# dmosopt/dmosopt

Hardware: NVIDIA H100
Metric: candidate-evals/sec (GP+sort+HV) pop=65536 dim=30 obj=3 (higher is better)
Workload: dtype f64 results; GP variance contraction in split-fp16 wgmma with fp32 accumulation (precision=auto: calibrated against the float64 path, 0 of 65535 rows of the last step recomputed in float64); ranks on u32 ids

## Files before the change

dmosopt_b200/csrc/common.cuh:

```cuda
#pragma once

#include <cuda_runtime.h>
#include <math.h>
#include <stdint.h>
#include <stdio.h>

#include <string>
#include <vector>

#include "../../include/dmosopt_b200.h"

struct dmo_ctx {
  int device = 0;
  cudaStream_t stream = nullptr;
  cudaMemPool_t pool = nullptr;
  cudaEvent_t ev0 = nullptr, ev1 = nullptr;
  int sm_count = 132;
  int64_t launches = 0;
  int64_t waits = 0;
  std::string err;
  void* flush_buf = nullptr;
  size_t flush_bytes = 0;
  int* dev_flag = nullptr;
  uint64_t h2d_bytes = 0, d2h_bytes = 0;
// ... 210 lines not shown
};
__device__ __forceinline__ double u01_53(uint32_t hi, uint32_t lo) {
  return (double)((((uint64_t)(hi >> 5)) << 26) | (uint64_t)(lo >> 6)) * (1.0 / 9007199254740992.0);
}

__device__ __forceinline__ double warp_sum(double v) {
#pragma unroll
  for (int o = 16; o > 0; o >>= 1) v += __shfl_xor_sync(0xffffffffu, v, o);
  return v;
}

template <int NW>
__device__ __forceinline__ double block_sum(double v, double* red) {
  v = warp_sum(v);
  __syncthreads();
  if ((threadIdx.x & 31) == 0) red[threadIdx.x >> 5] = v;
  __syncthreads();
  double s = 0.0;
#pragma unroll 8
  for (int w = 0; w < NW; ++w) s += red[w];
  __syncthreads();
  return s;
}

#endif

int prim_sort_pairs_u64(dmo_ctx* ctx, const uint64_t* kin, uint64_t* kout, const uint32_t* vin,
                        uint32_t* vout, int64_t n, int begin_bit, int end_bit);
int prim_sort_pairs_u32(dmo_ctx* ctx, const uint32_t* kin, uint32_t* kout, const uint32_t* vin,
                        uint32_t* vout, int64_t n, int begin_bit, int end_bit);
int prim_inclusive_sum_u32(dmo_ctx* ctx, const uint32_t* in, uint32_t* out, int64_t n);
int prim_exclusive_sum_i32(dmo_ctx* ctx, const int32_t* in, int32_t* out, int64_t n);
int prim_inclusive_min_f64(dmo_ctx* ctx, const double* in, double* out, int64_t n);
int prim_iota_u32(dmo_ctx* ctx, uint32_t* out, int64_t n);
int prim_gather_u32(dmo_ctx* ctx, const uint32_t* src, const uint32_t* idx, int64_t n, uint32_t* out);
int prim_round_f32(dmo_ctx* ctx, double* a, int64_t n);
int prim_col_keys(dmo_ctx* ctx, const double* dF, int64_t n, int M, int j, uint64_t* keys, uint32_t* idx);
int prim_sort_by_column(dmo_ctx* ctx, const double* dF, int64_t n, int M, int j, DevBuf<uint32_t>& sidx);

int rank_nd_device(dmo_ctx* ctx, const double* dY, int64_t n, int M, int32_t* d_rank);
int rank_nd_device_keep(dmo_ctx* ctx, const double* dY, int64_t n, int M, int64_t keep, int32_t* d_rank);
int nondominated_flags_device(dmo_ctx* ctx, const double* dY, int64_t n, int M, int32_t* d_flag01);
int nondominated_keep_flags(dmo_ctx* ctx, const double* dF, int64_t n, int M, DevBuf<int32_t>& flag);
int dense_ids(dmo_ctx* ctx, const double* dY, int64_t n, int M, DevBuf<uint32_t>& R, DevBuf<uint32_t>& maxid);
int lex_order(dmo_ctx* ctx, const uint32_t* R, int64_t n, int M, int sshift, DevBuf<uint32_t>& permA, DevBuf<uint32_t>& permB,
              const uint32_t** perm);
int crowding_device(dmo_ctx* ctx, const double* dY, int64_t n, int M, double* dD);
int euclidean_device(dmo_ctx* ctx, const double* dY, int64_t n, int M, double* dD);
int lexsort_device(dmo_ctx* ctx, const int32_t* d_rank, const double* const* d_desc_keys, int nkeys,
                   int64_t n, uint32_t* d_perm, bool rank_below_n);
int hypervolume_device(dmo_ctx* ctx, const double* dF, int64_t n, int M, const double* h_ref, double* h_out);
int hypervolume_device_ranked(dmo_ctx* ctx, const double* dF, int64_t n, int M, const double* h_ref, const int32_t* d_rank,
                              double* h_out);
int tournament_device(dmo_ctx* ctx, const int32_t* d_rank, const double* d_crowd, int64_t pop, int64_t poolsize, uint64_t seed,
                      uint64_t stream_id, int64_t* d_pool, double* d_u);
int nsga2_generate_device(dmo_ctx* ctx, const double* d_pop_x, int d, const int64_t* d_pool, int64_t poolsize, int64_t popsize,
                          double crossover_prob, double mutation_prob, double mutation_rate, const double* d_dic,
                          const double* d_dim, const double* d_xlb, const double* d_xub, uint64_t seed, uint64_t stream_id,
                          double* d_x_gen, int32_t* d_kind, int64_t* n_children, double* d_draws);
int remove_worst_device(dmo_ctx* ctx, const double* dX, const double* dY, int64_t n, int d, int M, int metric,
                        const double* const* d_extra, int n_extra, int64_t keep, double* dX_out, double* dY_out, int32_t* d_rank_out,
                        int64_t* d_perm_out);
int feas_rank_device(dmo_ctx* ctx, const dmo_feas* m, const double* dX, int64_t n, double* d_rank);
int feas_model_dim(const dmo_feas* m);
```

dmosopt_b200/csrc/gp.cuh:

```cuda
#pragma once
#include <vector>

#include "common.cuh"

struct GpVarOps {
  int64_t Npad = 0;
  int G = 0;
  std::vector<double> h_kscale;
  DevBuf<double> Linv;
  bool tensor_ready = false;
  DevBuf<uint16_t> Lhi, Llo;
  DevBuf<float> Lscale;
  DevBuf<int> Kexp;
  int alloc(dmo_ctx* ctx, int64_t N, int G);
};

struct dmo_gp {
  int64_t N = 0;
  int d = 0, M = 0, kernel = 0;
  bool isotropic = true;
  GpVarOps ops;
  std::vector<int> h_cov, h_lead;
  DevBuf<int> cov;
  DevBuf<double> Xt;
  DevBuf<double> alpha;
  DevBuf<double> inv_ls;
  DevBuf<double> g_inv_ls, g_constant;
  DevBuf<double> constant, noise, ymean, ystd;
  DevBuf<double> xlb, xrg;
  std::vector<double> h_constant, h_noise, h_ystd;
  bool has_linear_mean = false;
  DevBuf<double> lin_w, lin_b;
  DevBuf<float> Xtf;
  DevBuf<float> CAf;
  bool calibrated = false;
  bool auto_mean_tensor = false;
  bool auto_var_tensor = false;
  double cal_mean_err = 0.0;
  bool auto_mean_only = false;
  double cal_mean_err_only = 0.0;
  double cal_var_err = 0.0;
  double refine_theta = 1.0;
  int64_t last_refined = 0;
};

__device__ __forceinline__ double stationary(double s2, int kind) {
  if (kind == DMO_KERNEL_MATERN52) {
    const double K = sqrt(s2) * 2.23606797749978969641;
    return (1.0 + K + K * K / 3.0) * exp(-K);
  }
  return exp(-0.5 * s2);
}

constexpr int64_t GP_MAX_CHUNK = (int64_t)1 << 20;

int gp_predict_fp64(dmo_ctx* ctx, dmo_gp* gp, const double* dXn, int64_t P, double* d_mean, double* d_var);

int gp_linv_from_factor(dmo_ctx* ctx, const double* L, int64_t N, int64_t ldo, double* dst);
int gp_linv_from_factor_batched(dmo_ctx* ctx, const double* L, int64_t ldl, int64_t sL, int64_t N, int nbat, int64_t ldo,
                                int64_t sdst, double* dst);
int gp_fit_batched(dmo_ctx* ctx, int64_t N, int d, int nbat, int kernel, const double* X, const double* inv_ls, const double* constant,
                   const double* diag_add, const double* y, double* A, int64_t ld, int* info, double* work, double* alpha, double* lml);
int gp_potrf_batched(dmo_ctx* ctx, double* A, int64_t ld, int nbat, int* info);
constexpr int GP_F64_TILE = 128;
int gp_var_contract_fp64(dmo_ctx* ctx, const GpVarOps& ops, const double* Ks, int64_t kplane, int64_t Pcpad, int nsplit,
                         double* vnorm, int64_t vn_ld);
int gp_prepare_tensor(dmo_ctx* ctx, GpVarOps& ops);
constexpr int GP_TC_TILE = 128;
int gp_tensor_var_planes(int64_t Npad);
int gp_var_contract_tensor(dmo_ctx* ctx, const GpVarOps& ops, const uint16_t* Kh, const uint16_t* Kl, int64_t k_alloc,
                           int64_t k_rows, int64_t Pcpad, double* vnorm, int64_t vn_ld, int* abort_flag);
struct GpOverlap {
  cudaEvent_t mean_ready = nullptr;
};
int gp_predict_tensor(dmo_ctx* ctx, dmo_gp* gp, const double* dXn, int64_t P, double* d_mean, double* d_var,
                      int* abort_flag = nullptr, const GpOverlap* ov = nullptr);
extern const char* const GP_WATCHDOG_MSG;
struct GpPending {
  GpOverlap ov;
  bool active = false;
  int64_t P = 0;
  const double* dXn = nullptr;
  double *d_mean = nullptr, *d_var = nullptr;
  DevBuf<double> xn;
  DevBuf<int32_t> flag, pos;
};
int gp_predict_device(dmo_ctx* ctx, dmo_gp* gp, const double* dX, int64_t P, double* d_mean, double* d_var, int precision,
                      GpPending* pending = nullptr);
int gp_predict_finish(dmo_ctx* ctx, dmo_gp* gp, GpPending& pending, bool* refined);

struct GpUnitPredict {
  const char* who = "";
  bool tensor = false;
  int64_t tile = 0;
  int64_t Pc_alloc = 0;
  int n_vp = 0;
  DevBuf<double> vnorm, Ks;
  DevBuf<uint16_t> Kh, Kl;
  DevBuf<int> abort_flag;
  int check(dmo_ctx* ctx, const char* who, int precision, int d);
  int alloc(dmo_ctx* ctx, int64_t P, int64_t Npad, int planes, bool want_var);
  int contract(dmo_ctx* ctx, const GpVarOps& ops, int64_t Pcpad);
  int watchdog(dmo_ctx* ctx);
};

template <typename T>
int upload(dmo_ctx* ctx, DevBuf<T>& dst, const std::vector<T>& src) {
  DMO_TRY(dst.alloc(ctx, src.size()));
  DMO_CUDA(cudaMemcpyAsync(dst.p, src.data(), src.size() * sizeof(T), cudaMemcpyHostToDevice, ctx->stream));
  return DMO_OK;
}

int sv_gemm(dmo_ctx* ctx, int64_t m, int64_t n, int64_t K, double alpha, const double* A, int64_t sai, int64_t sak, const double* B,
            int64_t sbk, int64_t sbj, double diag, double* C, int64_t ldc);
int sv_flip(dmo_ctx* ctx, const double* C, int64_t n, double s, double* O, int64_t ldo);
int svgp_latent_moments(dmo_ctx* ctx, dmo_svgp* sv, GpUnitPredict& up, const double* X, int64_t P, double* fm, double* fv);
struct SvLatentView {
  const double *O0, *O1, *A, *XtT, *inv_ls;
  int64_t Npad;
};
int svgp_latent_view(const dmo_svgp* sv, int l, SvLatentView* v);

constexpr int MT_MAX = 8;
constexpr int MT_FIT_DMAX = 90;
// ... 26 lines not shown
```

dmosopt_b200/csrc/gp_tensor.cu:

```cuda
#include <cuda.h>
#include <cuda_fp16.h>
#include <cudaTypedefs.h>
#include <stdlib.h>

#include "gp.cuh"

namespace {

constexpr int TN = 256;
constexpr int TMV = 128;
constexpr int TK = 32;
constexpr int UK = 16;
constexpr int STAGES = 4;
constexpr int A_BYTES = TMV * TK * 2;
constexpr int B_BYTES = TN * TK * 2;
constexpr int STAGE_BYTES = 2 * A_BYTES + 2 * B_BYTES;
constexpr size_t GEMM_SMEM = (size_t)STAGES * STAGE_BYTES + 1024 + 256;
constexpr int NTHREADS = 384;

__device__ __forceinline__ uint32_t smem_u32(const void* p) { return (uint32_t)__cvta_generic_to_shared(p); }

__device__ __forceinline__ void mbar_init(uint64_t* bar, uint32_t count) {
  asm volatile("mbarrier.init.shared::cta.b64 [%0], %1;" ::"r"(smem_u32(bar)), "r"(count) : "memory");
}
// ... 846 lines not shown
#define KM_SWITCH(ISO_)        \
  switch (M) {                 \
    case 1: KM_LAUNCH(ISO_, 1); break; \
    case 2: KM_LAUNCH(ISO_, 2); break; \
    case 3: KM_LAUNCH(ISO_, 3); break; \
    case 4: KM_LAUNCH(ISO_, 4); break; \
    case 5: KM_LAUNCH(ISO_, 5); break; \
    default: KM_LAUNCH(ISO_, 6); break; \
  }
      if (gp->isotropic) {
        KM_SWITCH(true)
      } else {
        KM_SWITCH(false)
      }
#undef KM_SWITCH
#undef KM_LAUNCH
    }
    DMO_LAUNCH(mean_finish_tc_kernel, (unsigned)ceil_div(Pc * M, 256), 256, 0, mpart.p, (int)nsplit, Pc, ld, M, gp->ymean.p,
               gp->ystd.p, p_base, d_mean);
  }
  DMO_CHECK_LAUNCH();
  return DMO_OK;
}

}

int gp_prepare_tensor(dmo_ctx* ctx, GpVarOps& ops) {
  if (ops.tensor_ready) return DMO_OK;
  const int G = ops.G;
  const int64_t Npad = ops.Npad;
  std::vector<int> kexp(G);
  for (int g = 0; g < G; ++g) {
    double c = ops.h_kscale[g];
    kexp[g] = (c > 0.0) ? 13 - ilogb(c) : 13;
  }
  DMO_TRY(ops.Kexp.alloc(ctx, G));
  DMO_CUDA(cudaMemcpyAsync(ops.Kexp.p, kexp.data(), G * sizeof(int), cudaMemcpyHostToDevice, ctx->stream));
  DMO_CUDA(dmo_wait(ctx));
  DMO_TRY(ops.Lhi.alloc(ctx, (size_t)G * Npad * Npad));
  DMO_TRY(ops.Llo.alloc(ctx, (size_t)G * Npad * Npad));
  DMO_TRY(ops.Lscale.alloc(ctx, (size_t)G * Npad));
  DMO_LAUNCH(split_linv_kernel, (unsigned)(G * Npad), 256, 0, ops.Linv.p, Npad, ops.Kexp.p, ops.Lhi.p, ops.Llo.p,
             ops.Lscale.p);
  DMO_CHECK_LAUNCH();
  ops.tensor_ready = true;
  return DMO_OK;
}

static_assert(TMV == GP_TC_TILE, "gp.cuh exports the wgmma candidate tile");

int gp_tensor_var_planes(int64_t Npad) { return (int)((Npad / TN + 1) / 2); }

int gp_var_contract_tensor(dmo_ctx* ctx, const GpVarOps& ops, const uint16_t* Kh, const uint16_t* Kl, int64_t k_alloc,
                           int64_t k_rows, int64_t Pcpad, double* vnorm, int64_t vn_ld, int* abort_flag) {
  const int64_t Npad = ops.Npad;
  DMO_REQUIRE(Npad % TN == 0 && Pcpad % TMV == 0, "gp_var_contract_tensor: internal padding error");
  CUtensorMap map_kh, map_kl, map_lh, map_ll;
  DMO_TRY(make_map(ctx, &map_kh, Kh, (uint64_t)k_alloc, (uint64_t)Npad, TMV, TK, CU_TENSOR_MAP_SWIZZLE_64B));
  DMO_TRY(make_map(ctx, &map_kl, Kl, (uint64_t)k_alloc, (uint64_t)Npad, TMV, TK, CU_TENSOR_MAP_SWIZZLE_64B));
  DMO_TRY(make_map(ctx, &map_lh, ops.Lhi.p, (uint64_t)ops.G * Npad, (uint64_t)Npad, TN, TK, CU_TENSOR_MAP_SWIZZLE_64B));
  DMO_TRY(make_map(ctx, &map_ll, ops.Llo.p, (uint64_t)ops.G * Npad, (uint64_t)Npad, TN, TK, CU_TENSOR_MAP_SWIZZLE_64B));
  DMO_CUDA(cudaFuncSetAttribute(gp_var_wgmma_kernel, cudaFuncAttributeMaxDynamicSharedMemorySize, (int)GEMM_SMEM));
  GemmParams prm;
  prm.M = ops.G;
  prm.n_pb = (int)(Pcpad / TMV);
  prm.n_jt = (int)(Npad / TN);
  prm.n_q = gp_tensor_var_planes(Npad);
  prm.k_rows = k_rows;
  prm.l_rows = Npad;
  prm.inv_scale = ops.Lscale.p;
  prm.vnorm = vnorm;
  prm.vn_ld = vn_ld;
  prm.abort_flag = abort_flag;
  const int n_work = prm.M * prm.n_pb * prm.n_q;
  const int per_cta = (int)ceil_div(n_work, ctx->sm_count);
  const int grid = (int)ceil_div(n_work, per_cta);
  DMO_LAUNCH(gp_var_wgmma_kernel, grid, NTHREADS, GEMM_SMEM, map_kh, map_kl, map_lh, map_ll, prm);
  return DMO_OK;
}

const char* const GP_WATCHDOG_MSG = "gp_predict(tensor): pipeline watchdog tripped (mbarrier wait timed out)";

int gp_predict_tensor(dmo_ctx* ctx, dmo_gp* gp, const double* dXn, int64_t P, double* d_mean, double* d_var, int* abort_flag,
                      const GpOverlap* ov) {
  const int64_t N = gp->N, Npad = gp->ops.Npad;
  const int M = gp->M, G = gp->ops.G, d = gp->d;
  DMO_REQUIRE(M <= 16, "gp_predict(tensor): at most 16 objectives per model (got %d)", M);
  DMO_REQUIRE(d <= 64, "gp_predict(tensor): at most 64 input dimensions (got %d); use DMO_GP_FP64", d);
  DMO_REQUIRE(Npad % TN == 0, "gp_predict(tensor): internal padding error");
  if (!d_var && d <= KM_D && M <= 6)
    return gp_mean_direct(ctx, gp, dXn, P, d_mean);
  DMO_TRY(gp_prepare_tensor(ctx, gp->ops));
  constexpr int64_t TMv = KM_Q;
  int64_t Pc_max = ((int64_t)6 << 30) / ((int64_t)G * Npad * 4);
  if (Pc_max > GP_MAX_CHUNK) Pc_max = GP_MAX_CHUNK;
  Pc_max = (Pc_max / TMv) * TMv;
  if (Pc_max < TMv) Pc_max = TMv;
  const int64_t Pc_alloc = P < Pc_max ? ceil_div(P, TMv) * TMv : Pc_max;
  const int n_q = gp_tensor_var_planes(Npad);
  DevBuf<uint16_t> Kh, Kl;
  DevBuf<double> vnorm;
  DevBuf<int> own_flag;
  DMO_TRY(Kh.alloc(ctx, (size_t)G * Pc_alloc * Npad));
  DMO_TRY(Kl.alloc(ctx, (size_t)G * Pc_alloc * Npad));
  DMO_TRY(vnorm.alloc(ctx, (size_t)n_q * G * Pc_alloc));
  const bool read_back = abort_flag == nullptr;
  if (read_back) {
    DMO_TRY(own_flag.alloc(ctx, 1));
    abort_flag = own_flag.p;
  }
  DMO_CUDA(cudaMemsetAsync(abort_flag, 0, sizeof(int), ctx->stream));
  const int64_t kplane = Pc_alloc * Npad;
  const bool fused = d <= KM_D && M <= 6 && (gp->isotropic || G <= 2) &&
                     !(getenv("DMO_GP_FUSED") && atoi(getenv("DMO_GP_FUSED")) == 0);
  DevBuf<double> mpart;
  if (fused) DMO_TRY(prepare_direct_state(ctx, gp));
  for (int64_t p_base = 0; p_base < P; p_base += Pc_alloc) {
    const int64_t Pc = (P - p_base) < Pc_alloc ? (P - p_base) : Pc_alloc;
    const int64_t Pcpad = ceil_div(Pc, TMv) * TMv;
    if (fused) {
      int64_t n_per_block = Npad;
      const int64_t n_qb = Pcpad / KM_Q;
      const int64_t nsplit = pick_slices(n_qb, Npad, KF_NS, (int64_t)3 * ctx->sm_count, &n_per_block);
      DMO_TRY(mpart.alloc(ctx, (size_t)nsplit * M * Pcpad));
      dim3 gf((unsigned)nsplit, (unsigned)(Pcpad / KS_Q));
      const size_t smem = kstar_mean_smem(M);
      {
        ProfileScope ps_(ctx, "gp_kstar");
// ... 21 lines not shown
      case 4: KF_LAUNCH(ISO_, 4, false); break;                 \
      case 5: KF_LAUNCH(ISO_, 5, false); break;                 \
      default: KF_LAUNCH(ISO_, 6, false); break;                \
    }                                                           \
  }
        if (gp->isotropic) {
          KF_SWITCH(true)
        } else {
          KF_SWITCH(false)
        }
#undef KF_SWITCH
#undef KF_LAUNCH
      }
      DMO_LAUNCH(mean_finish_tc_kernel, (unsigned)ceil_div(Pc * M, 256), 256, 0, mpart.p, (int)nsplit, Pc, Pcpad, M, gp->ymean.p,
                 gp->ystd.p, p_base, d_mean);
    } else {
      {
        ProfileScope ps_(ctx, "gp_kstar");
        const int dmax = d <= 32 ? 32 : 64;
        size_t smem = (size_t)(KT_TP * dmax + G * dmax + G) * sizeof(float);
        dim3 gk((unsigned)(Npad / (2 * KT_TN)), (unsigned)ceil_div(Pcpad, KT_TP));
#define KSTAR_LAUNCH(ISO_, DM_)                                                                                          \
  DMO_LAUNCH((kstar_tensor_kernel<ISO_, DM_>), gk, KT_TN, smem, dXn, P, p_base, Pcpad, gp->Xt.p, N, d, G, gp->kernel, \
             gp->g_inv_ls.p, gp->g_constant.p, gp->ops.Kexp.p, Npad, kplane, Kh.p, Kl.p)
        if (gp->isotropic) {
          if (d <= 32)
            KSTAR_LAUNCH(true, 32);
          else
            KSTAR_LAUNCH(true, 64);
        } else {
          if (d <= 32)
            KSTAR_LAUNCH(false, 32);
          else
            KSTAR_LAUNCH(false, 64);
        }
#undef KSTAR_LAUNCH
      }
      {
        ProfileScope ps_(ctx, "gp_mean");
        DMO_LAUNCH(mean_split_kernel, (unsigned)ceil_div(Pc * M * 32, 256), 256, 0, Kh.p, Kl.p, Pc, N, Npad, kplane, M,
                   gp->cov.p, gp->ops.Kexp.p, gp->alpha.p, gp->ymean.p, gp->ystd.p, p_base, d_mean);
      }
    }
    if (ov && p_base + Pc_alloc >= P) DMO_CUDA(cudaEventRecord(ov->mean_ready, ctx->stream));
    if (d_var) {
      {
        ProfileScope ps_(ctx, "gp_var");
        cudaStream_t main = ctx->stream;
        if (ov) {
          DMO_CUDA(cudaEventRecord(ctx->lane_ev[1], main));
          DMO_CUDA(cudaStreamWaitEvent(ctx->gp_hi, ctx->lane_ev[1], 0));
          ctx->stream = ctx->gp_hi;
        }
        const int rc = gp_var_contract_tensor(ctx, gp->ops, Kh.p, Kl.p, G * Pc_alloc, Pc_alloc, Pcpad, vnorm.p, Pc_alloc, abort_flag);
        if (ov) {
          ctx->stream = main;
          DMO_CUDA(cudaEventRecord(ctx->lane_ev[2], ctx->gp_hi));
          DMO_CUDA(cudaStreamWaitEvent(main, ctx->lane_ev[2], 0));
        }
        DMO_TRY(rc);
      }
      DMO_LAUNCH(var_finish_tc_kernel, (unsigned)ceil_div(Pc * M, 256), 256, 0, vnorm.p, n_q, Pc, Pc_alloc, M, G,
                 gp->cov.p, gp->constant.p, gp->noise.p, gp->ystd.p, p_base, d_var);
    }
  }
  DMO_CHECK_LAUNCH();
  if (!read_back) return DMO_OK;
  int h_abort = 0;
  DMO_CUDA(cudaMemcpyAsync(&h_abort, abort_flag, sizeof(int), cudaMemcpyDeviceToHost, ctx->stream));
  DMO_CUDA(dmo_wait(ctx));
  if (h_abort) return dmo_fail(ctx, DMO_ERR_INTERNAL, "%s", GP_WATCHDOG_MSG);
  return DMO_OK;
}
```

dmosopt_b200/csrc/hv.cu:

```cuda
#include <stdlib.h>

#include "common.cuh"

int hv_many_device(dmo_ctx* ctx, const double* Fnd, const uint32_t* sidx, int64_t n, int M, const double* dref, double* h_out);
int hv3_tree_device(dmo_ctx* ctx, const double* xs, const double* ys, const double* zs, const uint32_t* zo, int64_t n, double rx,
                    double ry, double rz, double* partial, int64_t* n_partial);

namespace {

constexpr int HV_T = 128;

__global__ void inside_flag_kernel(const double* __restrict__ F, int64_t n, int M, const double* __restrict__ ref,
                                   const int32_t* __restrict__ drop, int32_t* __restrict__ flag) {
  int64_t i = (int64_t)blockIdx.x * blockDim.x + threadIdx.x;
  if (i > n) return;
  if (i == n) {
    flag[i] = 0;
    return;
  }
  bool in = drop == nullptr || drop[i] == 0;
  for (int j = 0; j < M; ++j) in = in && (ref[j] > F[i * M + j]);
  flag[i] = in ? 1 : 0;
}

__global__ void rank0_flag_kernel(const int32_t* __restrict__ rank, int64_t n, int32_t* __restrict__ flag) {
  int64_t i = (int64_t)blockIdx.x * blockDim.x + threadIdx.x;
  if (i > n) return;
  flag[i] = (i < n && rank[i] == 0) ? 1 : 0;
}

__global__ void compact_rows_kernel(const double* __restrict__ F, int64_t n, int M, const int32_t* __restrict__ flag,
                                    const int32_t* __restrict__ pos, double* __restrict__ out) {
  int64_t i = (int64_t)blockIdx.x * blockDim.x + threadIdx.x;
  if (i >= n || !flag[i]) return;
  for (int j = 0; j < M; ++j) out[(int64_t)pos[i] * M + j] = F[i * M + j];
}

__global__ void invert_perm_kernel(const uint32_t* __restrict__ sidx, int64_t n, uint32_t* __restrict__ inv) {
  int64_t p = (int64_t)blockIdx.x * blockDim.x + threadIdx.x;
  if (p < n) inv[sidx[p]] = (uint32_t)p;
}

__global__ void min_col_kernel(const double* __restrict__ F, int64_t n, double* out) {
  __shared__ double s[256];
  double m = INFINITY;
  for (int64_t i = threadIdx.x; i < n; i += blockDim.x) m = fmin(m, F[i]);
  s[threadIdx.x] = m;
  __syncthreads();
  for (int o = 128; o > 0; o >>= 1) {
    if (threadIdx.x < o) s[threadIdx.x] = fmin(s[threadIdx.x], s[threadIdx.x + o]);
    __syncthreads();
  }
  if (threadIdx.x == 0) out[0] = s[0];
// ... 322 lines not shown
                 int64_t* count) {
  DevBuf<int32_t> pos;
  DMO_TRY(pos.alloc(ctx, n + 1));
  DMO_TRY(prim_exclusive_sum_i32(ctx, flag.p, pos.p, n + 1));
  int32_t h = 0;
  DMO_CUDA(cudaMemcpyAsync(&h, pos.p + n, sizeof(int32_t), cudaMemcpyDeviceToHost, ctx->stream));
  DMO_CUDA(dmo_wait(ctx));
  *count = h;
  DMO_TRY(out.alloc(ctx, (size_t)(h > 0 ? h : 1) * M));
  if (h > 0) DMO_LAUNCH(compact_rows_kernel, (unsigned)ceil_div(n, 256), 256, 0, dF, n, M, flag.p, pos.p, out.p);
  DMO_CHECK_LAUNCH();
  return DMO_OK;
}

}

int nondominated_keep_flags(dmo_ctx* ctx, const double* dF, int64_t n, int M, DevBuf<int32_t>& flag) {
  DevBuf<uint32_t> sidx;
  DMO_TRY(flag.alloc(ctx, n + 1));
  if (n >= 1024) {
    DevBuf<int32_t> rank;
    DMO_TRY(rank.alloc(ctx, n));
    DMO_TRY(nondominated_flags_device(ctx, dF, n, M, rank.p));
    DMO_LAUNCH(rank0_flag_kernel, (unsigned)ceil_div(n + 1, 256), 256, 0, rank.p, n, flag.p);
    return DMO_OK;
  }
  DMO_TRY(prim_sort_by_column(ctx, dF, n, M, 0, sidx));
  {
    ProfileScope ps(ctx, "nd_filter");
    if (M <= 8)
      DMO_LAUNCH(nondominated_flag_kernel<8>, (unsigned)ceil_div(n, ND_T), ND_T, (size_t)ND_T * M * sizeof(double), dF, sidx.p, n, M,
                 flag.p);
    else
      DMO_LAUNCH(nondominated_flag_kernel<16>, (unsigned)ceil_div(n, ND_T), ND_T, (size_t)ND_T * M * sizeof(double), dF, sidx.p, n, M,
                 flag.p);
  }
  return DMO_OK;
}

namespace {

int nondominated_subset(dmo_ctx* ctx, const double* dF, int64_t n, int M, DevBuf<double>& out, int64_t* count) {
  DevBuf<int32_t> flag;
  DMO_TRY(nondominated_keep_flags(ctx, dF, n, M, flag));
  DMO_TRY(compact_rows(ctx, dF, n, M, flag, out, count));
  return DMO_OK;
}

__global__ void dominated_flag_kernel(const int32_t* __restrict__ keep, int64_t n, int32_t* __restrict__ out) {
  int64_t i = (int64_t)blockIdx.x * blockDim.x + threadIdx.x;
  if (i < n) out[i] = keep[i] ? 0 : 1;
}

int sum_partials(dmo_ctx* ctx, DevBuf<double>& partial, int64_t nb, double* h_out) {
  DevBuf<double> res;
  DMO_TRY(res.alloc(ctx, 1));
  DMO_LAUNCH(final_sum_kernel, 1, 256, 0, partial.p, nb, res.p);
  DMO_CHECK_LAUNCH();
  DMO_CUDA(cudaMemcpyAsync(h_out, res.p, sizeof(double), cudaMemcpyDeviceToHost, ctx->stream));
  DMO_CUDA(dmo_wait(ctx));
  return DMO_OK;
}

}

int hv_inside_nondominated(dmo_ctx* ctx, const double* dF, int64_t n, int M, const double* dref, DevBuf<double>& out,
                           int64_t* count) {
  *count = 0;
  DevBuf<int32_t> flag;
  DevBuf<double> Fin;
  int64_t n1 = 0;
  DMO_TRY(flag.alloc(ctx, n + 1));
  DMO_LAUNCH(inside_flag_kernel, (unsigned)ceil_div(n + 1, 256), 256, 0, dF, n, M, dref, (const int32_t*)nullptr, flag.p);
  DMO_TRY(compact_rows(ctx, dF, n, M, flag, Fin, &n1));
  if (n1 == 0) return DMO_OK;
  return nondominated_subset(ctx, Fin.p, n1, M, out, count);
}

int hypervolume_device_ranked(dmo_ctx* ctx, const double* dF, int64_t n, int M, const double* h_ref, const int32_t* d_rank,
                              double* h_out);

int hypervolume_device(dmo_ctx* ctx, const double* dF, int64_t n, int M, const double* h_ref, double* h_out) {
  return hypervolume_device_ranked(ctx, dF, n, M, h_ref, nullptr, h_out);
}

int hypervolume_device_ranked(dmo_ctx* ctx, const double* dF, int64_t n, int M, const double* h_ref, const int32_t* d_rank,
                              double* h_out) {
  *h_out = 0.0;
  if (n <= 0) return DMO_OK;
  DMO_REQUIRE(M >= 1 && M <= 8, "hypervolume: M=%d not supported (1..8; >= 10 objectives use Monte-Carlo in the reference)", M);
  DevBuf<double> dref;
  DMO_TRY(dref.alloc(ctx, M));
  DMO_CUDA(cudaMemcpyAsync(dref.p, h_ref, M * sizeof(double), cudaMemcpyHostToDevice, ctx->stream));
  DevBuf<int32_t> flag;
  DevBuf<double> Fin;
  int64_t n1 = 0;
  DMO_TRY(flag.alloc(ctx, n + 1));
  DMO_LAUNCH(inside_flag_kernel, (unsigned)ceil_div(n + 1, 256), 256, 0, dF, n, M, dref.p, d_rank, flag.p);
  DMO_TRY(compact_rows(ctx, dF, n, M, flag, Fin, &n1));
  if (n1 == 0) return DMO_OK;
  if (M == 1) {
    DevBuf<double> mn;
    DMO_TRY(mn.alloc(ctx, 1));
    DMO_LAUNCH(min_col_kernel, 1, 256, 0, Fin.p, n1, mn.p);
    DMO_CHECK_LAUNCH();
    double h = 0.0;
// ... 53 lines not shown
    for (int a = 0; a < D; ++a) {
      DMO_TRY(sc[a].alloc(ctx, n2));
      DMO_TRY(so_[a].alloc(ctx, n2));
      DMO_TRY(prim_sort_by_column(ctx, Fnd.p, n2, M, 2 + a, sidx_a));
      DMO_LAUNCH(invert_perm_kernel, g4, 256, 0, sidx_a.p, n2, inv_a.p);
      DMO_TRY(prim_gather_u32(ctx, inv_a.p, sx.p, n2, so_[a].p));
      DMO_LAUNCH(gather_col_kernel, g4, 256, 0, Fnd.p, sx.p, n2, M, 2 + a, sc[a].p);
      A.s[a] = sc[a].p;
      A.o[a] = so_[a].p;
      A.rs[a] = h_ref[2 + a];
    }
    const int64_t tiles = ceil_div(n2, HV_T);
    const int64_t nbv = ceil_div(n2, 256);
    DevBuf<double> part_main, part_a, part_b;
    DMO_TRY(part_main.alloc(ctx, (size_t)n2 * tiles));
    DMO_TRY(part_a.alloc(ctx, nbv));
    DMO_TRY(part_b.alloc(ctx, nbv));
    DMO_REQUIRE(tiles <= 65535, "hypervolume: front too large for M=%d (%lld non-dominated points)", M, (long long)n2);
    dim3 grid((unsigned)n2, (unsigned)tiles);
    double t_main = 0.0, t_a = 0.0, t_b = 0.0;
    {
      ProfileScope ps(ctx, M == 4 ? "hv4" : "hv5");
      if (M == 4) {
        DMO_LAUNCH(hv_slice_kernel<2>, grid, HV_T, 0, A, n2, part_main.p);
        DMO_LAUNCH(hv_volume_terms_kernel<2>, (unsigned)nbv, 256, 0, A, n2, part_a.p, part_b.p);
      } else {
        DMO_LAUNCH(hv_slice_kernel<3>, grid, HV_T, 0, A, n2, part_main.p);
        DMO_LAUNCH(hv_volume_terms_kernel<3>, (unsigned)nbv, 256, 0, A, n2, part_a.p, part_b.p);
      }
    }
    DMO_TRY(sum_partials(ctx, part_main, n2 * tiles, &t_main));
    DMO_TRY(sum_partials(ctx, part_a, nbv, &t_a));
    if (M == 5) DMO_TRY(sum_partials(ctx, part_b, nbv, &t_b));
    *h_out = (M == 4) ? (t_a - t_main) : (t_a - t_b + t_main);
    return DMO_OK;
  }
  DevBuf<uint32_t> sz, zinv, zo;
  DevBuf<double> xs, ys, zs;
  DMO_TRY(prim_sort_by_column(ctx, Fnd.p, n2, M, 2, sz));
  DMO_TRY(zinv.alloc(ctx, n2));
  DMO_TRY(zo.alloc(ctx, n2));
  DMO_TRY(xs.alloc(ctx, n2));
  DMO_TRY(ys.alloc(ctx, n2));
  DMO_TRY(zs.alloc(ctx, n2));
  const unsigned g = (unsigned)ceil_div(n2, 256);
  DMO_LAUNCH(invert_perm_kernel, g, 256, 0, sz.p, n2, zinv.p);
  DMO_TRY(prim_gather_u32(ctx, zinv.p, sx.p, n2, zo.p));
  DMO_LAUNCH(gather_col_kernel, g, 256, 0, Fnd.p, sx.p, n2, M, 0, xs.p);
  DMO_LAUNCH(gather_col_kernel, g, 256, 0, Fnd.p, sx.p, n2, M, 1, ys.p);
  DMO_LAUNCH(gather_col_kernel, g, 256, 0, Fnd.p, sx.p, n2, M, 2, zs.p);
  int64_t nb = ceil_div(n2, HV_T);
  DevBuf<double> partial;
  DMO_TRY(partial.alloc(ctx, nb));
  int64_t tree_min = 4096;
  if (const char* e = getenv("DMO_HV3_TREE")) {
    const long v = atol(e);
    tree_min = v == 0 ? INT64_MAX : (v == 1 ? 0 : v);
  }
  if (n2 >= tree_min) {
    DMO_TRY(hv3_tree_device(ctx, xs.p, ys.p, zs.p, zo.p, n2, h_ref[0], h_ref[1], h_ref[2], partial.p, &nb));
  } else {
    ProfileScope ps(ctx, "hv3");
    DMO_LAUNCH(hv3_kernel, (unsigned)nb, HV_T, 0, xs.p, ys.p, zs.p, zo.p, n2, h_ref[0], h_ref[1], h_ref[2], partial.p);
  }
  DMO_TRY(sum_partials(ctx, partial, nb, h_out));
  return DMO_OK;
}

extern "C" {

int dmo_hypervolume(dmo_ctx* ctx, const double* F, int64_t n, int M, const double* ref, double* out) {
  if (!ctx) return DMO_ERR_ARG;
  DMO_CUDA(cudaSetDevice(ctx->device));
  DMO_REQUIRE(out && ref && n >= 0 && M >= 1 && M <= 16, "hypervolume: bad arguments");
  *out = 0.0;
  if (n == 0) return DMO_OK;
  DMO_REQUIRE(F, "hypervolume: null points");
  double h_ref[16];
  DMO_CUDA(cudaMemcpy(h_ref, ref, M * sizeof(double), cudaMemcpyDefault));
  In<double> f;
  DMO_TRY(f.init(ctx, F, (size_t)n * M));
  DMO_TRY(hypervolume_device(ctx, f.d, n, M, h_ref, out));
  return DMO_OK;
}

int dmo_nondominated_flags(dmo_ctx* ctx, const double* Y, int64_t n, int M, int32_t* flags) {
  if (!ctx) return DMO_ERR_ARG;
  DMO_CUDA(cudaSetDevice(ctx->device));
  DMO_REQUIRE(n >= 0 && M >= 1 && M <= 16, "nondominated_flags: bad shape n=%lld M=%d", (long long)n, M);
  if (n == 0) return DMO_OK;
  DMO_REQUIRE(Y && flags, "nondominated_flags: null pointer");
  In<double> y;
  Out<int32_t> f;
  DMO_TRY(y.init(ctx, Y, (size_t)n * M));
  DMO_TRY(f.init(ctx, flags, (size_t)n));
  DevBuf<int32_t> keep;
  DMO_TRY(nondominated_keep_flags(ctx, y.d, n, M, keep));
  DMO_LAUNCH(dominated_flag_kernel, (unsigned)ceil_div(n, 256), 256, 0, keep.p, n, f.d);
  DMO_CHECK_LAUNCH();
  DMO_TRY(f.finish(ctx));
  DMO_CUDA(dmo_wait(ctx));
  return DMO_OK;
}

int dmo_hypervolume_ranked(dmo_ctx* ctx, const double* F, int64_t n, int M, const double* ref, const int32_t* rank,
                           double* out) {
  if (!ctx) return DMO_ERR_ARG;
  DMO_CUDA(cudaSetDevice(ctx->device));
  DMO_REQUIRE(out && ref && n >= 0 && M >= 1 && M <= 16, "hypervolume_ranked: bad arguments");
  *out = 0.0;
  if (n == 0) return DMO_OK;
  DMO_REQUIRE(F && rank, "hypervolume_ranked: null points / ranks");
  double h_ref[16];
  DMO_CUDA(cudaMemcpy(h_ref, ref, M * sizeof(double), cudaMemcpyDefault));
  In<double> f;
  In<int32_t> r;
  DMO_TRY(f.init(ctx, F, (size_t)n * M));
  DMO_TRY(r.init(ctx, rank, (size_t)n));
  DMO_TRY(hypervolume_device_ranked(ctx, f.d, n, M, h_ref, r.d, out));
// ... 71 lines not shown
```

dmosopt_b200/csrc/step.cu:

```cuda
#include <string.h>

#include <algorithm>

#include "common.cuh"
#include "gp.cuh"

constexpr int kCountWarps = 8;
__global__ void __launch_bounds__(kCountWarps * 32) step_counts_kernel(const int32_t* __restrict__ kind, int64_t P,
                                                                        const int64_t* __restrict__ perm, int64_t pop,
                                                                        unsigned long long* counts) {
  __shared__ double red[kCountWarps];
  double c[4] = {0.0, 0.0, 0.0, 0.0};
  const int64_t n = P > pop ? P : pop;
  for (int64_t i = (int64_t)blockIdx.x * blockDim.x + threadIdx.x; i < n; i += (int64_t)gridDim.x * blockDim.x) {
    if (i < P) {
      const int32_t k = kind[i];
      c[0] += k < 2 ? 1.0 : 0.0;
      c[1] += k == 2 ? 1.0 : 0.0;
    }
    if (i < pop) {
      const int64_t j = perm[i];
      if (j < P) {
        const int32_t k = kind[j];
        c[2] += k < 2 ? 1.0 : 0.0;
        c[3] += k == 2 ? 1.0 : 0.0;
      }
    }
  }
#pragma unroll
  for (int k = 0; k < 4; ++k) {
    const double s = block_sum<kCountWarps>(c[k], red);
    if (threadIdx.x == 0 && s > 0.0) atomicAdd(&counts[k], (unsigned long long)s);
  }
}

static int copy_out(dmo_ctx* ctx, void* dst, const void* src, size_t bytes) {
  cudaPointerAttributes a;
  if (cudaPointerGetAttributes(&a, dst) != cudaSuccess) {
    cudaGetLastError();
    a.type = cudaMemoryTypeUnregistered;
  }
  if (a.type == cudaMemoryTypeUnregistered) ctx->waits++;
  if (a.type != cudaMemoryTypeDevice && a.type != cudaMemoryTypeManaged) ctx->d2h_bytes += bytes;
  DMO_CUDA(cudaMemcpyAsync(dst, src, bytes, cudaMemcpyDefault, ctx->stream));
  return DMO_OK;
}

static int nsga2_step_body(dmo_ctx* ctx, dmo_gp* gp, const dmo_feas* key, double* pop_x, double* pop_y, int32_t* rank,
                           int64_t pop, int d, int M, double crossover_prob, double mutation_prob, double mutation_rate,
                           const double* di_crossover, const double* di_mutation, const double* xlb, const double* xub,
                           uint64_t seed, uint64_t stream_id, int precision, int distance_metric, int with_variance,
                           int round_to_f32, const double* hv_ref, int64_t* n_children, double* hv_out, double* x_gen,
                           double* y_gen, int64_t* counts) {
  if (!ctx) return DMO_ERR_ARG;
  DMO_CUDA(cudaSetDevice(ctx->device));
  DMO_REQUIRE(gp && pop_x && pop_y && rank && pop >= 2 && d >= 1 && M >= 1 && di_crossover && di_mutation && xlb && xub,
              "nsga2_step: bad arguments");
  DMO_REQUIRE(distance_metric == DMO_METRIC_NONE || distance_metric == DMO_METRIC_CROWDING || distance_metric == DMO_METRIC_EUCLIDEAN,
              "nsga2_step: unknown distance metric %d", distance_metric);
  DMO_REQUIRE(dmo_is_device_ptr(pop_x) && dmo_is_device_ptr(pop_y) && dmo_is_device_ptr(rank),
              "nsga2_step: the population (pop_x, pop_y, rank) must be resident on the device");
  int64_t poolsize = pop / 2;
  if ((pop & 1) && (poolsize & 1)) poolsize += 1;
  const int64_t cap = pop + 1;
  DevBuf<int64_t> pool, perm;
  DevBuf<double> Xs, Ys, var;
  DevBuf<int32_t> kind;
  DMO_TRY(pool.alloc(ctx, poolsize));
  DMO_TRY(perm.alloc(ctx, pop));
  DMO_TRY(Xs.alloc(ctx, (size_t)(cap + pop) * d));
  DMO_TRY(Ys.alloc(ctx, (size_t)(cap + pop) * M));
  DMO_TRY(kind.alloc(ctx, cap));
  if (with_variance) DMO_TRY(var.alloc(ctx, (size_t)cap * M));
  In<double> idc, idm, ilb, iub;
  DMO_TRY(idc.init(ctx, di_crossover, d));
  DMO_TRY(idm.init(ctx, di_mutation, d));
  DMO_TRY(ilb.init(ctx, xlb, d));
  DMO_TRY(iub.init(ctx, xub, d));
  {
    ProfileScope ps(ctx, "step_tournament");
    DMO_TRY(tournament_device(ctx, rank, nullptr, pop, poolsize, seed, stream_id, pool.p, nullptr));
  }
  int64_t P = 0;
  {
    ProfileScope ps(ctx, "step_generate");
    DMO_TRY(nsga2_generate_device(ctx, pop_x, d, pool.p, poolsize, pop, crossover_prob, mutation_prob, mutation_rate, idc.d, idm.d,
                                  ilb.d, iub.d, seed, stream_id + 1, Xs.p, kind.p, &P, nullptr));
  }
  if (n_children) *n_children = P;
  {
    ProfileScope ps(ctx, "step_truncate");
    DMO_CUDA(cudaMemcpyAsync(Xs.p + (size_t)P * d, pop_x, (size_t)pop * d * sizeof(double), cudaMemcpyDeviceToDevice, ctx->stream));
    DMO_CUDA(cudaMemcpyAsync(Ys.p + (size_t)P * M, pop_y, (size_t)pop * M * sizeof(double), cudaMemcpyDeviceToDevice, ctx->stream));
  }
  DevBuf<double> kx;
  const double* kp[1] = {nullptr};
  if (key) {
    ProfileScope ps(ctx, "step_truncate");
    DMO_TRY(kx.alloc(ctx, (size_t)(P + pop)));
    DMO_TRY(feas_rank_device(ctx, key, Xs.p, P + pop, kx.p));
    kp[0] = kx.p;
  }
  GpPending gpp;
  DevBuf<int32_t> rank_in;
  if (P > 0) {
    DMO_TRY(rank_in.alloc(ctx, pop));
    DMO_TRY(dmo_lane_streams(ctx));
    gpp.ov.mean_ready = ctx->lane_ev[0];
    ProfileScope ps(ctx, "step_gp");
    DMO_TRY(gp_predict_device(ctx, gp, Xs.p, P, Ys.p, with_variance ? var.p : nullptr, precision, &gpp));
  }
  auto truncate = [&]() -> int {
    ProfileScope ps(ctx, "step_truncate");
    DMO_TRY(remove_worst_device(ctx, Xs.p, Ys.p, P + pop, d, M, distance_metric, key ? kp : nullptr, key ? 1 : 0, pop, pop_x, pop_y,
                                rank, perm.p));
    if (round_to_f32) DMO_TRY(prim_round_f32(ctx, pop_y, pop * M));
    return DMO_OK;
  };
  auto first_truncate = [&]() -> int {
    if (gpp.active) DMO_CUDA(cudaMemcpyAsync(rank_in.p, rank, (size_t)pop * sizeof(int32_t), cudaMemcpyDeviceToDevice, ctx->stream));
    return truncate();
  };
  if (gpp.active && gpp.ov.mean_ready) {
    cudaStream_t main = ctx->stream;
    DMO_CUDA(cudaStreamWaitEvent(ctx->lane, gpp.ov.mean_ready, 0));
    ctx->stream = ctx->lane;
    const int rc = first_truncate();
    ctx->stream = main;
    DMO_CUDA(cudaEventRecord(ctx->lane_ev[3], ctx->lane));
    DMO_CUDA(cudaStreamWaitEvent(main, ctx->lane_ev[3], 0));
    DMO_TRY(rc);
  } else {
    DMO_TRY(first_truncate());
  }
  bool refined = false;
  const int rc = gp_predict_finish(ctx, gp, gpp, &refined);
  if (rc != DMO_OK) {
    DMO_CUDA(cudaMemcpyAsync(pop_x, Xs.p + (size_t)P * d, (size_t)pop * d * sizeof(double), cudaMemcpyDeviceToDevice, ctx->stream));
    DMO_CUDA(cudaMemcpyAsync(pop_y, Ys.p + (size_t)P * M, (size_t)pop * M * sizeof(double), cudaMemcpyDeviceToDevice, ctx->stream));
    DMO_CUDA(cudaMemcpyAsync(rank, rank_in.p, (size_t)pop * sizeof(int32_t), cudaMemcpyDeviceToDevice, ctx->stream));
    DMO_CUDA(dmo_wait(ctx));
    return rc;
  }
  if (refined) DMO_TRY(truncate());
  if (x_gen) {
    ProfileScope ps(ctx, "step_record");
    DevBuf<unsigned long long> cnt;
    DMO_TRY(cnt.alloc(ctx, 4));
    DMO_CUDA(cudaMemsetAsync(cnt.p, 0, 4 * sizeof(unsigned long long), ctx->stream));
    const int64_t n = P > pop ? P : pop;
    const unsigned grid = (unsigned)std::min<int64_t>(ceil_div(n, kCountWarps * 32), 4 * (int64_t)ctx->sm_count);
    DMO_LAUNCH(step_counts_kernel, grid, kCountWarps * 32, 0, kind.p, P, perm.p, pop, cnt.p);
    DMO_CHECK_LAUNCH();
    DMO_TRY(copy_out(ctx, x_gen, Xs.p, (size_t)P * d * sizeof(double)));
    DMO_TRY(copy_out(ctx, y_gen, Ys.p, (size_t)P * M * sizeof(double)));
    DMO_TRY(copy_out(ctx, counts, cnt.p, 4 * sizeof(int64_t)));
  }
  if (hv_ref && hv_out) {
    ProfileScope ps(ctx, "step_hv");
    DMO_REQUIRE(M <= 16, "nsga2_step: too many objectives for the hypervolume");
    double h_ref[16];
    if (dmo_is_device_ptr(hv_ref)) {
      ctx->waits++;
      DMO_CUDA(cudaMemcpyAsync(h_ref, hv_ref, M * sizeof(double), cudaMemcpyDeviceToHost, ctx->stream));
    } else {
      memcpy(h_ref, hv_ref, M * sizeof(double));
    }
    DMO_TRY(hypervolume_device_ranked(ctx, pop_y, pop, M, h_ref, rank, hv_out));
  }
  return DMO_OK;
}

extern "C" {
int dmo_nsga2_step(dmo_ctx* ctx, dmo_gp* gp, double* pop_x, double* pop_y, int32_t* rank, int64_t pop, int d, int M,
                   double crossover_prob, double mutation_prob, double mutation_rate, const double* di_crossover,
                   const double* di_mutation, const double* xlb, const double* xub, uint64_t seed, uint64_t stream_id,
                   int precision, int distance_metric, int with_variance, int round_to_f32, const double* hv_ref, int64_t* n_children,
                   double* hv_out) {
  return nsga2_step_body(ctx, gp, nullptr, pop_x, pop_y, rank, pop, d, M, crossover_prob, mutation_prob, mutation_rate,
                         di_crossover, di_mutation, xlb, xub, seed, stream_id, precision, distance_metric, with_variance,
                         round_to_f32, hv_ref, n_children, hv_out, nullptr, nullptr, nullptr);
}

int dmo_nsga2_step_record(dmo_ctx* ctx, dmo_gp* gp, const dmo_feas* key, double* pop_x, double* pop_y, int32_t* rank,
                          int64_t pop, int d, int M, double crossover_prob, double mutation_prob, double mutation_rate,
                          const double* di_crossover, const double* di_mutation, const double* xlb, const double* xub,
                          uint64_t seed, uint64_t stream_id, int precision, int distance_metric, int round_to_f32,
                          double* x_gen, double* y_gen, int64_t* counts, int64_t* n_children) {
  if (!ctx) return DMO_ERR_ARG;
  DMO_REQUIRE(x_gen && y_gen && counts, "nsga2_step_record: x_gen, y_gen and counts are required");
  DMO_REQUIRE(!key || feas_model_dim(key) == d, "nsga2_step_record: the key model takes %d columns, the population has %d",
              feas_model_dim(key), d);
  return nsga2_step_body(ctx, gp, key, pop_x, pop_y, rank, pop, d, M, crossover_prob, mutation_prob, mutation_rate,
                         di_crossover, di_mutation, xlb, xub, seed, stream_id, precision, distance_metric, 0, round_to_f32,
                         nullptr, n_children, nullptr, x_gen, y_gen, counts);
}
}
```

Measured before the change: 8.797 million.

## Overlap 3-objective hypervolume with GP variance on side lane, reserve SMs

Moves the ranked 3-objective hypervolume preparation (compaction, sorts, gathers, and the tree pass when large) onto the side lane stream, right after the first truncation. It then runs concurrently with the GP variance contraction, and only a small finish step runs afterwards. The wgmma variance kernel now sizes its grid to leave a configurable number of SMs free when overlap is active, so the lane work can make progress. This costs extra work for the variance GEMM on fewer SMs, and the speculative HV work is discarded if refinement retruncates. It also pads unused rows with the reference point so sizes are fixed before the inside count is known.

```diff
diff --git a/dmosopt_b200/csrc/common.cuh b/dmosopt_b200/csrc/common.cuh
--- a/dmosopt_b200/csrc/common.cuh
+++ b/dmosopt_b200/csrc/common.cuh
@@ -286,6 +286,16 @@
 int hypervolume_device(dmo_ctx* ctx, const double* dF, int64_t n, int M, const double* h_ref, double* h_out);
 int hypervolume_device_ranked(dmo_ctx* ctx, const double* dF, int64_t n, int M, const double* h_ref, const int32_t* d_rank,
                               double* h_out);
+struct Hv3Ranked {
+  int64_t n = 0;
+  double ref[3] = {0.0, 0.0, 0.0};
+  bool tree = false;
+  DevBuf<int32_t> pos;
+  DevBuf<double> xs, ys, zs, res;
+  DevBuf<uint32_t> zo;
+};
+int hv3_ranked_enqueue(dmo_ctx* ctx, const double* dF, int64_t n, const double* h_ref, const int32_t* d_rank, Hv3Ranked& s);
+int hv3_ranked_finish(dmo_ctx* ctx, Hv3Ranked& s, double* h_out);
 int tournament_device(dmo_ctx* ctx, const int32_t* d_rank, const double* d_crowd, int64_t pop, int64_t poolsize, uint64_t seed,
                       uint64_t stream_id, int64_t* d_pool, double* d_u);
 int nsga2_generate_device(dmo_ctx* ctx, const double* d_pop_x, int d, const int64_t* d_pool, int64_t poolsize, int64_t popsize,
diff --git a/dmosopt_b200/csrc/gp.cuh b/dmosopt_b200/csrc/gp.cuh
--- a/dmosopt_b200/csrc/gp.cuh
+++ b/dmosopt_b200/csrc/gp.cuh
@@ -69,7 +69,11 @@
 constexpr int GP_TC_TILE = 128;
 int gp_tensor_var_planes(int64_t Npad);
 int gp_var_contract_tensor(dmo_ctx* ctx, const GpVarOps& ops, const uint16_t* Kh, const uint16_t* Kl, int64_t k_alloc,
-                           int64_t k_rows, int64_t Pcpad, double* vnorm, int64_t vn_ld, int* abort_flag);
+                           int64_t k_rows, int64_t Pcpad, double* vnorm, int64_t vn_ld, int* abort_flag, int free_sms = 0);
+#ifndef DMO_GP_LANE_SMS
+#define DMO_GP_LANE_SMS 14
+#endif
+constexpr int GP_LANE_SMS = DMO_GP_LANE_SMS;
 struct GpOverlap {
   cudaEvent_t mean_ready = nullptr;
 };
diff --git a/dmosopt_b200/csrc/gp_tensor.cu b/dmosopt_b200/csrc/gp_tensor.cu
--- a/dmosopt_b200/csrc/gp_tensor.cu
+++ b/dmosopt_b200/csrc/gp_tensor.cu
@@ -922,7 +922,7 @@
 int gp_tensor_var_planes(int64_t Npad) { return (int)((Npad / TN + 1) / 2); }
 
 int gp_var_contract_tensor(dmo_ctx* ctx, const GpVarOps& ops, const uint16_t* Kh, const uint16_t* Kl, int64_t k_alloc,
-                           int64_t k_rows, int64_t Pcpad, double* vnorm, int64_t vn_ld, int* abort_flag) {
+                           int64_t k_rows, int64_t Pcpad, double* vnorm, int64_t vn_ld, int* abort_flag, int free_sms) {
   const int64_t Npad = ops.Npad;
   DMO_REQUIRE(Npad % TN == 0 && Pcpad % TMV == 0, "gp_var_contract_tensor: internal padding error");
   CUtensorMap map_kh, map_kl, map_lh, map_ll;
@@ -943,7 +943,7 @@
   prm.vn_ld = vn_ld;
   prm.abort_flag = abort_flag;
   const int n_work = prm.M * prm.n_pb * prm.n_q;
-  const int per_cta = (int)ceil_div(n_work, ctx->sm_count);
+  const int per_cta = (int)ceil_div(n_work, ctx->sm_count - free_sms > 1 ? ctx->sm_count - free_sms : 1);
   const int grid = (int)ceil_div(n_work, per_cta);
   DMO_LAUNCH(gp_var_wgmma_kernel, grid, NTHREADS, GEMM_SMEM, map_kh, map_kl, map_lh, map_ll, prm);
   return DMO_OK;
@@ -1071,7 +1071,8 @@
           DMO_CUDA(cudaStreamWaitEvent(ctx->gp_hi, ctx->lane_ev[1], 0));
           ctx->stream = ctx->gp_hi;
         }
-        const int rc = gp_var_contract_tensor(ctx, gp->ops, Kh.p, Kl.p, G * Pc_alloc, Pc_alloc, Pcpad, vnorm.p, Pc_alloc, abort_flag);
+        const int rc = gp_var_contract_tensor(ctx, gp->ops, Kh.p, Kl.p, G * Pc_alloc, Pc_alloc, Pcpad, vnorm.p, Pc_alloc, abort_flag,
+                                              ov ? GP_LANE_SMS : 0);
         if (ov) {
           ctx->stream = main;
           DMO_CUDA(cudaEventRecord(ctx->lane_ev[2], ctx->gp_hi));
diff --git a/dmosopt_b200/csrc/hv.cu b/dmosopt_b200/csrc/hv.cu
--- a/dmosopt_b200/csrc/hv.cu
+++ b/dmosopt_b200/csrc/hv.cu
@@ -1,4 +1,5 @@
 #include <stdlib.h>
+#include <string.h>
 
 #include "common.cuh"
 
@@ -427,6 +428,21 @@
   if (i < n) out[i] = keep[i] ? 0 : 1;
 }
 
+int64_t hv3_tree_min() {
+  if (const char* e = getenv("DMO_HV3_TREE")) {
+    const long v = atol(e);
+    return v == 0 ? INT64_MAX : (v == 1 ? 0 : v);
+  }
+  return 4096;
+}
+
+__global__ void pad_rows_kernel(double* __restrict__ F, int64_t n, int M, const int32_t* __restrict__ count,
+                                const double* __restrict__ ref) {
+  const int64_t i = (int64_t)blockIdx.x * blockDim.x + threadIdx.x;
+  if (i >= *count && i < n)
+    for (int j = 0; j < M; ++j) F[i * M + j] = ref[j];
+}
+
 int sum_partials(dmo_ctx* ctx, DevBuf<double>& partial, int64_t nb, double* h_out) {
   DevBuf<double> res;
   DMO_TRY(res.alloc(ctx, 1));
@@ -586,12 +602,7 @@
   int64_t nb = ceil_div(n2, HV_T);
   DevBuf<double> partial;
   DMO_TRY(partial.alloc(ctx, nb));
-  int64_t tree_min = 4096;
-  if (const char* e = getenv("DMO_HV3_TREE")) {
-    const long v = atol(e);
-    tree_min = v == 0 ? INT64_MAX : (v == 1 ? 0 : v);
-  }
-  if (n2 >= tree_min) {
+  if (n2 >= hv3_tree_min()) {
     DMO_TRY(hv3_tree_device(ctx, xs.p, ys.p, zs.p, zo.p, n2, h_ref[0], h_ref[1], h_ref[2], partial.p, &nb));
   } else {
     ProfileScope ps(ctx, "hv3");
@@ -599,6 +610,69 @@
   }
   DMO_TRY(sum_partials(ctx, partial, nb, h_out));
   return DMO_OK;
+}
+
+int hv3_ranked_enqueue(dmo_ctx* ctx, const double* dF, int64_t n, const double* h_ref, const int32_t* d_rank, Hv3Ranked& s) {
+  s.n = n;
+  memcpy(s.ref, h_ref, sizeof(s.ref));
+  s.tree = n >= hv3_tree_min();
+  DevBuf<double> dref, Fin;
+  DevBuf<int32_t> flag;
+  DevBuf<uint32_t> sx, sz, zinv;
+  DMO_TRY(dref.alloc(ctx, 3));
+  DMO_CUDA(cudaMemcpyAsync(dref.p, h_ref, 3 * sizeof(double), cudaMemcpyHostToDevice, ctx->stream));
+  DMO_TRY(flag.alloc(ctx, n + 1));
+  DMO_TRY(s.pos.alloc(ctx, n + 1));
+  DMO_TRY(Fin.alloc(ctx, (size_t)n * 3));
+  const unsigned g = (unsigned)ceil_div(n, 256);
+  DMO_LAUNCH(inside_flag_kernel, (unsigned)ceil_div(n + 1, 256), 256, 0, dF, n, 3, dref.p, d_rank, flag.p);
+  DMO_TRY(prim_exclusive_sum_i32(ctx, flag.p, s.pos.p, n + 1));
+  DMO_LAUNCH(compact_rows_kernel, g, 256, 0, dF, n, 3, flag.p, s.pos.p, Fin.p);
+  DMO_LAUNCH(pad_rows_kernel, g, 256, 0, Fin.p, n, 3, s.pos.p + n, dref.p);
+  DMO_TRY(prim_sort_by_column(ctx, Fin.p, n, 3, 0, sx));
+  DMO_TRY(prim_sort_by_column(ctx, Fin.p, n, 3, 2, sz));
+  DMO_TRY(zinv.alloc(ctx, n));
+  DMO_TRY(s.zo.alloc(ctx, n));
+  DMO_TRY(s.xs.alloc(ctx, n));
+  DMO_TRY(s.ys.alloc(ctx, n));
+  DMO_TRY(s.zs.alloc(ctx, n));
+  DMO_LAUNCH(invert_perm_kernel, g, 256, 0, sz.p, n, zinv.p);
+  DMO_TRY(prim_gather_u32(ctx, zinv.p, sx.p, n, s.zo.p));
+  DMO_LAUNCH(gather_col_kernel, g, 256, 0, Fin.p, sx.p, n, 3, 0, s.xs.p);
+  DMO_LAUNCH(gather_col_kernel, g, 256, 0, Fin.p, sx.p, n, 3, 1, s.ys.p);
+  DMO_LAUNCH(gather_col_kernel, g, 256, 0, Fin.p, sx.p, n, 3, 2, s.zs.p);
+  if (s.tree) {
+    DevBuf<double> partial;
+    int64_t nb = ceil_div(n, HV_T);
+    DMO_TRY(partial.alloc(ctx, nb));
+    DMO_TRY(hv3_tree_device(ctx, s.xs.p, s.ys.p, s.zs.p, s.zo.p, n, h_ref[0], h_ref[1], h_ref[2], partial.p, &nb));
+    DMO_TRY(s.res.alloc(ctx, 1));
+    DMO_LAUNCH(final_sum_kernel, 1, 256, 0, partial.p, nb, s.res.p);
+  }
+  DMO_CHECK_LAUNCH();
+  return DMO_OK;
+}
+
+int hv3_ranked_finish(dmo_ctx* ctx, Hv3Ranked& s, double* h_out) {
+  *h_out = 0.0;
+  int32_t n1 = 0;
+  DMO_CUDA(cudaMemcpyAsync(&n1, s.pos.p + s.n, sizeof(int32_t), cudaMemcpyDeviceToHost, ctx->stream));
+  DMO_CUDA(dmo_wait(ctx));
+  if (n1 == 0) return DMO_OK;
+  if (s.tree && n1 >= hv3_tree_min()) {
+    DMO_CUDA(cudaMemcpyAsync(h_out, s.res.p, sizeof(double), cudaMemcpyDeviceToHost, ctx->stream));
+    DMO_CUDA(dmo_wait(ctx));
+    return DMO_OK;
+  }
+  const int64_t nb = ceil_div(n1, HV_T);
+  DevBuf<double> partial;
+  DMO_TRY(partial.alloc(ctx, nb));
+  {
+    ProfileScope ps(ctx, "hv3");
+    DMO_LAUNCH(hv3_kernel, (unsigned)nb, HV_T, 0, s.xs.p, s.ys.p, s.zs.p, s.zo.p, (int64_t)n1, s.ref[0], s.ref[1], s.ref[2],
+               partial.p);
+  }
+  return sum_partials(ctx, partial, nb, h_out);
 }
 
 extern "C" {
diff --git a/dmosopt_b200/csrc/step.cu b/dmosopt_b200/csrc/step.cu
--- a/dmosopt_b200/csrc/step.cu
+++ b/dmosopt_b200/csrc/step.cu
@@ -1,6 +1,7 @@
 #include <string.h>
 
 #include <algorithm>
+#include <cmath>
 
 #include "common.cuh"
 #include "gp.cuh"
@@ -101,6 +102,16 @@
     DMO_TRY(feas_rank_device(ctx, key, Xs.p, P + pop, kx.p));
     kp[0] = kx.p;
   }
+  const bool want_hv = hv_ref && hv_out;
+  double h_ref[16] = {};
+  if (want_hv && M <= 16) {
+    if (dmo_is_device_ptr(hv_ref)) {
+      ctx->waits++;
+      DMO_CUDA(cudaMemcpyAsync(h_ref, hv_ref, M * sizeof(double), cudaMemcpyDeviceToHost, ctx->stream));
+    } else {
+      memcpy(h_ref, hv_ref, M * sizeof(double));
+    }
+  }
   GpPending gpp;
   DevBuf<int32_t> rank_in;
   if (P > 0) {
@@ -121,11 +132,23 @@
     if (gpp.active) DMO_CUDA(cudaMemcpyAsync(rank_in.p, rank, (size_t)pop * sizeof(int32_t), cudaMemcpyDeviceToDevice, ctx->stream));
     return truncate();
   };
+  auto hypervolume = [&](double* h) -> int {
+    ProfileScope ps(ctx, "step_hv");
+    return hypervolume_device_ranked(ctx, pop_y, pop, M, h_ref, rank, h);
+  };
+  Hv3Ranked hv_lane;
+  const bool hv_on_lane = want_hv && M == 3 && std::isfinite(h_ref[0]) && std::isfinite(h_ref[1]) && std::isfinite(h_ref[2]);
+  bool hv_enqueued = false;
   if (gpp.active && gpp.ov.mean_ready) {
     cudaStream_t main = ctx->stream;
     DMO_CUDA(cudaStreamWaitEvent(ctx->lane, gpp.ov.mean_ready, 0));
     ctx->stream = ctx->lane;
-    const int rc = first_truncate();
+    int rc = first_truncate();
+    if (rc == DMO_OK && hv_on_lane) {
+      ProfileScope ps(ctx, "step_hv");
+      rc = hv3_ranked_enqueue(ctx, pop_y, pop, h_ref, rank, hv_lane);
+      hv_enqueued = rc == DMO_OK;
+    }
     ctx->stream = main;
     DMO_CUDA(cudaEventRecord(ctx->lane_ev[3], ctx->lane));
     DMO_CUDA(cudaStreamWaitEvent(main, ctx->lane_ev[3], 0));
@@ -142,7 +165,10 @@
     DMO_CUDA(dmo_wait(ctx));
     return rc;
   }
-  if (refined) DMO_TRY(truncate());
+  if (refined) {
+    DMO_TRY(truncate());
+    hv_enqueued = false;
+  }
   if (x_gen) {
     ProfileScope ps(ctx, "step_record");
     DevBuf<unsigned long long> cnt;
@@ -156,17 +182,16 @@
     DMO_TRY(copy_out(ctx, y_gen, Ys.p, (size_t)P * M * sizeof(double)));
     DMO_TRY(copy_out(ctx, counts, cnt.p, 4 * sizeof(int64_t)));
   }
-  if (hv_ref && hv_out) {
-    ProfileScope ps(ctx, "step_hv");
+  if (want_hv) {
+    if (hv_enqueued) {
+      ProfileScope ps(ctx, "step_hv");
+      double h = 0.0;
+      DMO_TRY(hv3_ranked_finish(ctx, hv_lane, &h));
+      *hv_out = h;
+      return DMO_OK;
+    }
     DMO_REQUIRE(M <= 16, "nsga2_step: too many objectives for the hypervolume");
-    double h_ref[16];
-    if (dmo_is_device_ptr(hv_ref)) {
-      ctx->waits++;
-      DMO_CUDA(cudaMemcpyAsync(h_ref, hv_ref, M * sizeof(double), cudaMemcpyDeviceToHost, ctx->stream));
-    } else {
-      memcpy(h_ref, hv_ref, M * sizeof(double));
-    }
-    DMO_TRY(hypervolume_device_ranked(ctx, pop_y, pop, M, h_ref, rank, hv_out));
+    DMO_TRY(hypervolume(hv_out));
   }
   return DMO_OK;
 }
```

Result: faster. 9.209 million, median of 6 (+4.7%).
